# qwerty35/swarm_simulator

Measured on AMD Instinct MI355X. Metric: agent-trajectories/sec (RBP plan: SFC+RSFC+QP), higher is better.
Workload: dtype f64

## Files before the change

### swarm_simulator_amd/csrc/kernels/lh_inverse.inc

```
#define LH_H 3
#include "lh_layout.h"
#define LHP_ZERO 1

__device__ __forceinline__ void lhv_load(const double* x, double (&r)[LH_H], int nP, int lane) {
#pragma unroll
    for (int h = 0; h < LH_H; ++h) r[h] = lane + 64 * h < nP ? x[lane + 64 * h] : 0.0;
}
__device__ __forceinline__ void lhv_store(double* x, const double (&r)[LH_H], int nP, int lane) {
#pragma unroll
    for (int h = 0; h < LH_H; ++h)
        if (lane + 64 * h < nP) x[lane + 64 * h] = r[h];
}
struct LhV {
    double v[LH_H];
};
__device__ __forceinline__ double lhv_pick(const LhV& x, int h) { return h == 0 ? x.v[0] : (h == 1 ? x.v[1] : x.v[2]); }

template <class PT>
__device__ __noinline__ void lh_clear(PT W, int rows_v) {
    const int rows = __builtin_amdgcn_readfirstlane(rows_v);
    const int n = lhp_size(rows);
    for (int i = threadIdx.x & 63; i < n; i += 64) W[i] = 0.0;
    WSYNC();
}

template <int NH, class PT>
__device__ __forceinline__ void w_cols_span(PT W, const LhV& x, double (&out)[LH_H], int g0, int g1, int lane) {
    double A[8][NH], B[8][NH];
    auto load = [&](int g, double (&buf)[8][NH]) {
        const int L = lhp_len(g), base = lhp_grp(g);
#pragma unroll
        for (int h = 0; h < NH; ++h) {
            const int c = lane + 64 * h;
            if (c < L) {
#pragma unroll
                for (int u = 0; u < 8; ++u) buf[u][h] = W[base + u * (L + 1) + c];
            }
        }
    };
    auto use = [&](int g, const double (&buf)[8][NH]) {
        const int L = lhp_len(g);
        const double xs = lhv_pick(x, g >> 3);
        double xb[8];
#pragma unroll
        for (int u = 0; u < 8; ++u) xb[u] = rl_dyn(xs, (8 * g + u) & 63);
#pragma unroll
        for (int h = 0; h < NH; ++h) {
            if (lane + 64 * h < L) {
#pragma unroll
                for (int u = 0; u < 8; ++u) out[h] += buf[u][h] * xb[u];
            }
        }
    };
    if (g0 >= g1) return;
    load(g0, A);
    for (int g = g0; g < g1; g += 2) {
        if (g + 1 < g1) load(g + 1, B);
        use(g, A);
        if (g + 1 < g1) {
            if (g + 2 < g1) load(g + 2, A);
            use(g + 1, B);
        }
    }
}
template <int HM, class PT>
__device__ __noinline__ LhV w_cols_fn(PT W, LhV x, int nP_v) {
    const int nP = __builtin_amdgcn_readfirstlane(nP_v);
    const int lane = threadIdx.x & 63, ng = (nP + 7) >> 3;
    LhV o;
#pragma unroll
    for (int h = 0; h < LH_H; ++h) o.v[h] = 0.0;
    w_cols_span<1, PT>(W, x, o.v, 0, ng < 8 ? ng : 8, lane);
    if (ng > 8) w_cols_span<2, PT>(W, x, o.v, 8, ng < 16 ? ng : 16, lane);
    if (HM > 2 && ng > 16) w_cols_span<(HM > 2 ? 3 : 2), PT>(W, x, o.v, 16, ng, lane);
    return o;
}

template <class PT>
__device__ __noinline__ double w_cols1_fn(PT W, double x0, int nP_v) {
    const int nP = __builtin_amdgcn_readfirstlane(nP_v);
    LhV x, o;
    x.v[0] = x0, x.v[1] = x.v[2] = 0.0;
    o.v[0] = o.v[1] = o.v[2] = 0.0;
    w_cols_span<1, PT>(W, x, o.v, 0, (nP + 7) >> 3, threadIdx.x & 63);
    return o.v[0];
}

template <int H0, int HM, class PT>
__device__ __forceinline__ void w_rows_span(PT W, const LhV& x, double (&out)[LH_H], int g0, int g1, int nP, int lane) {
    constexpr int NH = HM - H0;
    int off[NH], row[NH];
#pragma unroll
    for (int q = 0; q < NH; ++q) {
        const int b = lane + 64 * (H0 + q);
        row[q] = b < nP ? b : -1;
        off[q] = lhp_row(b < nP ? b : 0);
    }
    double A[8][NH], B[8][NH];
    auto load = [&](int g, double (&buf)[8][NH]) {
#pragma unroll
        for (int q = 0; q < NH; ++q) {
            if (row[q] >= 8 * g) {
#pragma unroll
                for (int u = 0; u < 8; ++u) buf[u][q] = W[off[q] + 8 * g + u];
            }
        }
    };
    auto use = [&](int g, const double (&buf)[8][NH]) {
        const double xs = lhv_pick(x, g >> 3);
        double xc[8];
#pragma unroll
        for (int u = 0; u < 8; ++u) xc[u] = rl_dyn(xs, (8 * g + u) & 63);
#pragma unroll
        for (int q = 0; q < NH; ++q) {
            if (row[q] >= 8 * g) {
#pragma unroll
                for (int u = 0; u < 8; ++u) out[H0 + q] += buf[u][q] * xc[u];
            }
        }
    };
    if (g0 >= g1) return;
    load(g0, A);
    for (int g = g0; g < g1; g += 2) {
        if (g + 1 < g1) load(g + 1, B);
        use(g, A);
        if (g + 1 < g1) {
            if (g + 2 < g1) load(g + 2, A);
            use(g + 1, B);
        }
    }
}
template <int HM, class PT>
__device__ __noinline__ LhV w_rows_fn(PT W, LhV x, int nP_v) {
    const int nP = __builtin_amdgcn_readfirstlane(nP_v);
    const int lane = threadIdx.x & 63, ng = (nP + 7) >> 3;
    LhV o;
#pragma unroll
    for (int h = 0; h < LH_H; ++h) o.v[h] = 0.0;
    w_rows_span<0, HM, PT>(W, x, o.v, 0, ng < 8 ? ng : 8, nP, lane);
    if (ng > 8) w_rows_span<1, HM, PT>(W, x, o.v, 8, ng < 16 ? ng : 16, nP, lane);
    if (HM > 2 && ng > 16) w_rows_span<(HM > 2 ? 2 : 1), HM, PT>(W, x, o.v, 16, ng, nP, lane);
    return o;
}
template <class PT>
__device__ __noinline__ double w_rows1_fn(PT W, double x0, int nP_v) {
    const int nP = __builtin_amdgcn_readfirstlane(nP_v);
    const int lane = threadIdx.x & 63, ng = (nP + 7) >> 3;
    const int row = lane < nP ? lane : -1, off = lhp_row(lane < nP ? lane : 0);
    double out = 0.0;
    double A[8], B[8];
    auto load = [&](int g, double (&buf)[8]) {
        if (row >= 8 * g) {
#pragma unroll
            for (int u = 0; u < 8; ++u) buf[u] = W[off + 8 * g + u];
        }
    };
    auto use = [&](int g, const double (&buf)[8]) {
        double xc[8];
#pragma unroll
        for (int u = 0; u < 8; ++u) xc[u] = rl_dyn(x0, 8 * g + u);
        if (row >= 8 * g) {
#pragma unroll
            for (int u = 0; u < 8; ++u) out += buf[u] * xc[u];
        }
    };
    if (ng == 0) return 0.0;
    load(0, A);
    for (int g = 0; g < ng; g += 2) {
        if (g + 1 < ng) load(g + 1, B);
        use(g, A);
        if (g + 1 < ng) {
            if (g + 2 < ng) load(g + 2, A);
            use(g + 1, B);
        }
    }
    return out;
}

template <int H, class PT>
__device__ __noinline__ void w_delete_fn(PT W, double* scr_g, int nP_v, int k_v) {
    const int nP = __builtin_amdgcn_readfirstlane(nP_v), k = __builtin_amdgcn_readfirstlane(k_v);
    const int lane = threadIdx.x & 63;
    kl_lds* scr = (kl_lds*)scr_g;
    double cr[H];
#pragma unroll
    for (int h = 0; h < H; ++h) {
        const int b = lane + 64 * h;
        const bool on = b >= k && b < nP;
        const double v = W[on ? lhp_row(b) + k : LHP_ZERO];
        cr[h] = v;
        if (b < nP) scr[b] = v * v;
    }
    WSYNC();
    double cs[H], sn[H];
    {
        double run[H], prev[H];
#pragma unroll
        for (int h = 0; h < H; ++h) run[h] = 0.0, prev[h] = 0.0;
        for (int r0 = k; r0 < nP; r0 += 8) {
            double q[8];
#pragma unroll
            for (int u = 0; u < 8; ++u) q[u] = scr[r0 + u < nP ? r0 + u : k];
#pragma unroll
            for (int u = 0; u < 8; ++u) {
                const int r = r0 + u < nP ? r0 + u : 1 << 20;
#pragma unroll
                for (int h = 0; h < H; ++h) {
                    run[h] += r <= lane + 64 * h ? q[u] : 0.0;
                    prev[h] += r < lane + 64 * h ? q[u] : 0.0;
                }
            }
        }
#pragma unroll
        for (int h = 0; h < H; ++h) {
            const int i = lane + 64 * h;
            const bool on = i > k && i < nP;
            const double r2 = on ? run[h] : 1.0, p2 = on ? prev[h] : 1.0;
            const double inv = fast_rsqrt(r2);
            cs[h] = on ? p2 * fast_rsqrt(p2) * inv : 1.0;
            sn[h] = on ? cr[h] * inv : 0.0;
        }
    }
    constexpr int DU = 4;
    double acc[H], A[DU][H], B[DU][H];
    int cdst[H];
    auto fetch = [&](int i0, double (&g)[DU][H]) {
#pragma unroll
        for (int u = 0; u < DU; ++u) {
            const int i = i0 + u < nP ? i0 + u : nP - 1;
            const int off = lhp_row(i), len = lhp_len(i >> 3);
#pragma unroll
            for (int h = 0; h < H; ++h) g[u][h] = W[lane + 64 * h < len ? off + lane + 64 * h : LHP_ZERO];
        }
    };
    auto rotate = [&](int i0, const double (&g)[DU][H]) {
#pragma unroll
        for (int u = 0; u < DU; ++u) {
            const int i = i0 + u;
            if (i < nP) {
                const int li = i & 63, hi = i >> 6;
                double ci = rl_dyn(cs[0], li), si = rl_dyn(sn[0], li);
                if (H > 1 && hi == 1) ci = rl_dyn(cs[H > 1 ? 1 : 0], li), si = rl_dyn(sn[H > 1 ? 1 : 0], li);
                if (H > 2 && hi == 2) ci = rl_dyn(cs[H > 2 ? 2 : 0], li), si = rl_dyn(sn[H > 2 ? 2 : 0], li);
                const int tdst = lhp_row(i - 1), ldst = lhp_len((i - 1) >> 3);
#pragma unroll
                for (int h = 0; h < H; ++h) {
                    const double a = acc[h], rv = g[u][h];
                    acc[h] = ci * a + si * rv;
                    const double nv = ci * rv - si * a;
                    if (cdst[h] < ldst) W[tdst + cdst[h]] = nv;
                }
            }
        }
    };
#pragma unroll
    for (int h = 0; h < H; ++h) {
        const int c = lane + 64 * h;
        acc[h] = W[c < lhp_len(k >> 3) ? lhp_row(k) + c : LHP_ZERO];
        cdst[h] = c < k ? c : (c > k ? c - 1 : 1 << 20);
    }
    fetch(k + 1, A);
    for (int i0 = k + 1; i0 < nP; i0 += 2 * DU) {
        if (i0 + DU < nP) fetch(i0 + DU, B);
        rotate(i0, A);
        if (i0 + DU < nP) {
            if (i0 + 2 * DU < nP) fetch(i0 + 2 * DU, A);
            rotate(i0 + DU, B);
        }
    }
    WSYNC();
}

__device__ __forceinline__ void lh_rows(kl_lds* Wl, double* Wg, const double (&x)[LH_H], double (&out)[LH_H], int nP, int lane) {
    if (nP <= 64) {
        out[0] = Wg ? w_rows1_fn<double*>(Wg, x[0], nP) : w_rows1_fn<kl_lds*>(Wl, x[0], nP);
        out[1] = out[2] = 0.0;
        return;
    }
    LhV xi, o;
#pragma unroll
    for (int h = 0; h < LH_H; ++h) xi.v[h] = x[h];
    o = Wg ? w_rows_fn<3, double*>(Wg, xi, nP) : (nP <= 128 ? w_rows_fn<2, kl_lds*>(Wl, xi, nP) : w_rows_fn<3, kl_lds*>(Wl, xi, nP));
#pragma unroll
    for (int h = 0; h < LH_H; ++h) out[h] = o.v[h];
}
__device__ __forceinline__ void lh_cols(kl_lds* Wl, double* Wg, const double (&x)[LH_H], double (&out)[LH_H], int nP, int lane) {
    if (nP <= 64) {
        out[0] = Wg ? w_cols1_fn<double*>(Wg, x[0], nP) : w_cols1_fn<kl_lds*>(Wl, x[0], nP);
        out[1] = out[2] = 0.0;
        return;
    }
    LhV xi, o;
#pragma unroll
    for (int h = 0; h < LH_H; ++h) xi.v[h] = x[h];
    o = Wg ? w_cols_fn<3, double*>(Wg, xi, nP) : (nP <= 128 ? w_cols_fn<2, kl_lds*>(Wl, xi, nP) : w_cols_fn<3, kl_lds*>(Wl, xi, nP));
#pragma unroll
    for (int h = 0; h < LH_H; ++h) out[h] = o.v[h];
}
__device__ __forceinline__ void lh_delete(kl_lds* Wl, double* Wg, double* scr, int nP, int k, int lane) {
    if (Wg)
        w_delete_fn<3, double*>(Wg, scr, nP, k);
    else if (nP <= 64)
        w_delete_fn<1, kl_lds*>(Wl, scr, nP, k);
    else if (nP <= 128)
        w_delete_fn<2, kl_lds*>(Wl, scr, nP, k);
    else
        w_delete_fn<3, kl_lds*>(Wl, scr, nP, k);
}
__device__ __forceinline__ void lh_reset(kl_lds* Wl, double* Wg, int rows) {
    if (Wg)
        lh_clear<double*>(Wg, rows);
    else
        lh_clear<kl_lds*>(Wl, rows);
}
```

### swarm_simulator_amd/csrc/kernels/qp_polish.inc

```

__device__ __forceinline__ int cand_meta(const Cand& c) {
    return c.a | ((c.b + 1) << 8) | ((c.n[0] != 0.0) << 16) | ((c.n[1] != 0.0) << 17) | ((c.n[2] != 0.0) << 18);
}
__device__ __forceinline__ int meta_sign(int meta, int agent, int k) {
    if (!(((meta >> 16) >> k) & 1)) return 0;
    return agent == (meta & 255) ? 1 : (agent == ((meta >> 8) & 255) - 1 ? -1 : 0);
}
__device__ __forceinline__ double cand_dot(const Cand& c, const double* vec, int nk) {
    const double* blk = vec + (size_t)(c.knot - 1) * nk;
    double s = 0;
#pragma unroll
    for (int k = 0; k < 3; ++k) {
        if (c.n[k] == 0.0) continue;
        const double* pa = blk + (c.a * 3 + k) * 3;
        double ta = c.t[0] * pa[0] + c.t[1] * pa[1] + c.t[2] * pa[2];
        if (c.b >= 0) {
            const double* pb = blk + (c.b * 3 + k) * 3;
            ta -= c.t[0] * pb[0] + c.t[1] * pb[1] + c.t[2] * pb[2];
        }
        s += c.n[k] * ta;
    }
    return s;
}

__device__ void k0_mission_tables(int nj, const QpWs& w, const PolishWs& pw, double* lds) {
    double* f3 = lds;
    dd* fd = (dd*)(lds + 18 * nj);
    for (int it = threadIdx.x; it < 18 * nj; it += QP_THREADS) {
        const int jj = it / 18, e = it % 18, j = jj + 1;
        const double v = e < 9 ? w.Dk[9 * j + e] : (jj + 1 < nj ? w.Ek[9 * j + (e - 9)] : 0.0);
        f3[it] = v, fd[it] = dd(v);
    }
    __syncthreads();
    if (threadIdx.x == 0) {
        int ok = 1;
        double Bp[9] = {0, 0, 0, 0, 0, 0, 0, 0, 0};
        for (int jj = 0; jj < nj; ++jj)
            if (!k0_factor_step(f3 + 18 * jj, Bp, jj == 0)) ok = 0;
        *(int*)(pw.k0f + 18 * (size_t)nj) = !ok;
    }
    if (threadIdx.x == 64) {
        int ok = 1;
        dd Bd[9];
        for (int jj = 0; jj < nj; ++jj)
            if (!k0_factor_step(fd + 18 * jj, Bd, jj == 0)) ok = 0;
        *((int*)(pw.k0f + 18 * (size_t)nj) + 1) = !ok;
    }
    __syncthreads();
    for (int it = threadIdx.x; it < 18 * nj; it += QP_THREADS) pw.k0f[it] = f3[it];
    for (int col = threadIdx.x; col < 3 * nj; col += QP_THREADS) k0_inverse_column((const dd*)fd, nj, col / 3, col % 3, pw.G, pw.Sg);
    __threadfence_block();
    __syncthreads();
    for (int jj = threadIdx.x; jj < nj; jj += QP_THREADS) k0g_symmetrise(pw.G + k0g_block(jj, jj));
}

__device__ __forceinline__ void k0_solve3(const double* f3g, int nj, int nk, double* col, int sub) {
    typedef __attribute__((address_space(1))) double gdb;
    const kl_lds* f3 = (const kl_lds*)f3g;
    gdb* y = QG(col) + sub * 3;
    constexpr int B = K0_BLK;
    double cur[B][3], nxt[B][3];
    double p[3] = {0, 0, 0};
#pragma unroll
    for (int u = 0; u < B; ++u) {
        const int jx = u < nj ? u : nj - 1;
#pragma unroll
        for (int e = 0; e < 3; ++e) cur[u][e] = y[(size_t)jx * nk + e];
    }
    for (int j0 = 0; j0 < nj; j0 += B) {
#pragma unroll
        for (int u = 0; u < B; ++u) {
            const int jx = j0 + B + u < nj ? j0 + B + u : nj - 1;
#pragma unroll
            for (int e = 0; e < 3; ++e) nxt[u][e] = y[(size_t)jx * nk + e];
        }
#pragma unroll
        for (int u = 0; u < B; ++u) {
            const int jj = j0 + u;
            if (jj < nj) {
                k0_forward_step(f3 + 18 * jj, jj > 0, cur[u], p);
                y[(size_t)jj * nk] = p[0] = cur[u][0], y[(size_t)jj * nk + 1] = p[1] = cur[u][1], y[(size_t)jj * nk + 2] = p[2] = cur[u][2];
            }
        }
#pragma unroll
        for (int u = 0; u < B; ++u)
#pragma unroll
            for (int e = 0; e < 3; ++e) cur[u][e] = nxt[u][e];
    }
#pragma unroll
    for (int u = 0; u < B; ++u) {
        const int jx = nj - 1 - u >= 0 ? nj - 1 - u : 0;
#pragma unroll
        for (int e = 0; e < 3; ++e) cur[u][e] = y[(size_t)jx * nk + e];
    }
    for (int jt = nj - 1; jt >= 0; jt -= B) {
#pragma unroll
        for (int u = 0; u < B; ++u) {
            const int jx = jt - B - u >= 0 ? jt - B - u : 0;
#pragma unroll
            for (int e = 0; e < 3; ++e) nxt[u][e] = y[(size_t)jx * nk + e];
        }
#pragma unroll
        for (int u = 0; u < B; ++u) {
            const int jj = jt - u;
            if (jj >= 0) {
                k0_backward_step(f3 + 18 * jj, jj + 1 < nj, cur[u], p);
                y[(size_t)jj * nk] = p[0] = cur[u][0], y[(size_t)jj * nk + 1] = p[1] = cur[u][1], y[(size_t)jj * nk + 2] = p[2] = cur[u][2];
            }
        }
#pragma unroll
        for (int u = 0; u < B; ++u)
#pragma unroll
            for (int e = 0; e < 3; ++e) cur[u][e] = nxt[u][e];
    }
}

__device__ __noinline__ void v0_solve3_fn(int nj_v, int nk_v, int nb_v, double* v0_v, const double* f3_v) {
    const int nj = __builtin_amdgcn_readfirstlane(nj_v), nk = __builtin_amdgcn_readfirstlane(nk_v), nb = __builtin_amdgcn_readfirstlane(nb_v);
    double* v0 = uni(v0_v);
    const double* f3 = uni(f3_v);
    for (int it = threadIdx.x; it < nb * 3; it += QP_THREADS) k0_solve3(f3, nj, nk, v0, it);
}

__device__ __noinline__ void table_product_fn(int nj_v, int nk_v, int nb_v, const double* G_v, const double* u_v, double* out_v) {
    typedef __attribute__((address_space(1))) const double gcd;
    const int nj = __builtin_amdgcn_readfirstlane(nj_v), nk = __builtin_amdgcn_readfirstlane(nk_v), nsub = 3 * __builtin_amdgcn_readfirstlane(nb_v);
    gcd* G = QGC(uni(G_v));
    gcd* uv = QGC(uni(u_v));
    double* out = uni(out_v);
    constexpr int PB = 4;
    for (int it = threadIdx.x; it < nj * nsub; it += QP_THREADS) {
        const int jj = it / nsub, sub = it % nsub;
        double acc[3] = {0, 0, 0};
        for (int k0 = 0; k0 < nj; k0 += PB) {
            double g[PB][9], x[PB][3];
#pragma unroll
            for (int u = 0; u < PB; ++u) {
                const int kb = k0 + u < nj ? k0 + u : nj - 1;
                gcd* blk = G + (jj >= kb ? k0g_block(jj, kb) : k0g_block(kb, jj));
#pragma unroll
                for (int e = 0; e < 9; ++e) g[u][e] = blk[e];
#pragma unroll
                for (int e = 0; e < 3; ++e) x[u][e] = uv[(size_t)kb * nk + sub * 3 + e];
            }
#pragma unroll
            for (int u = 0; u < PB; ++u) {
                if (k0 + u >= nj) continue;
                if (jj >= k0 + u) {
                    acc[0] += g[u][0] * x[u][0] + g[u][1] * x[u][1] + g[u][2] * x[u][2];
                    acc[1] += g[u][3] * x[u][0] + g[u][4] * x[u][1] + g[u][5] * x[u][2];
                    acc[2] += g[u][6] * x[u][0] + g[u][7] * x[u][1] + g[u][8] * x[u][2];
                } else {
                    acc[0] += g[u][0] * x[u][0] + g[u][3] * x[u][1] + g[u][6] * x[u][2];
                    acc[1] += g[u][1] * x[u][0] + g[u][4] * x[u][1] + g[u][7] * x[u][2];
                    acc[2] += g[u][2] * x[u][0] + g[u][5] * x[u][1] + g[u][8] * x[u][2];
                }
            }
        }
        const size_t i = (size_t)jj * nk + sub * 3;
#pragma unroll
        for (int e = 0; e < 3; ++e) out[i + e] = -acc[e];
    }
}

__device__ __forceinline__ double s_from_table(const Cand* cand, const double* G, int ci, int cj, int ma, int mb) {
    const int aa = ma & 255, ab = ((ma >> 8) & 255) - 1, ba = mb & 255, bb = ((mb >> 8) & 255) - 1;
    const int sg = (aa == ba) - (bb >= 0 && aa == bb) - (ab >= 0 && ab == ba) + (ab >= 0 && ab == bb);
    bool share = aa == ba || (bb >= 0 && aa == bb) || (ab >= 0 && (ab == ba || ab == bb));
    if (share && ab < 0 && bb < 0) share = ((ma & mb) >> 16) != 0;
    if (!share || sg == 0) return 0.0;
    const Cand& ca = cand[ci];
    const Cand& cb = cand[cj];
    const bool a_first = ca.knot >= cb.knot;
    const double* blk = G + k0g_block((a_first ? ca.knot : cb.knot) - 1, (a_first ? cb.knot : ca.knot) - 1);
    return (double)sg * (ca.n[0] * cb.n[0] + ca.n[1] * cb.n[1] + ca.n[2] * cb.n[2]) * k0g_bilinear(blk, a_first, ca.t, cb.t);
}

__device__ __forceinline__ double rl_dyn(double v, int lane) {
    const int lo = __builtin_amdgcn_readlane(__double2loint(v), lane);
    const int hi = __builtin_amdgcn_readlane(__double2hiint(v), lane);
    return __hiloint2double(hi, lo);
}

#include "lh_inverse.inc"

__device__ int lh_wave(int n, const double* Sg, int ldS, const double* dv, double* zc, double* tv, double* yv, double* wv, int* P, int* inP,
                       int* banned, double* Lc, int* shared_int, int pmax, double* str, bool big, double* stats = nullptr, int resume_nP = -1,
                       int n_prev = 0) {
    const int lane = threadIdx.x & 63;
    kl_lds* Wl = big ? nullptr : (kl_lds*)Lc;
    double* Wg = big ? Lc : nullptr;
    int* rem = (int*)tv;
    int nP = 0;
    double dmax = 0;
    const bool resume = resume_nP >= 0;
    for (int a = lane; a < n; a += 64) {
        if (!resume || a >= n_prev)
            zc[a] = 0;
        else
            zc[a] = fmax(zc[a], 0.0);
        inP[a] = 0, banned[a] = 0;
        dmax = fmax(dmax, fabs(dv[a]));
    }
    dmax = wave_red(dmax, 1);
    const double wtol = 1e-12 * fmax(1.0, dmax);
    if (resume) {
        nP = resume_nP;
        WSYNC();
        for (int b = lane; b < nP; b += 64) inP[P[b]] = 1;
    } else {
        lh_reset(Wl, Wg, pmax);
    }
    WSYNC();
    bool warming = str != nullptr && !resume;
    bool w_valid = resume ? shared_int[1] != 0 : true;
    bool first_resumed = resume && nP > 0;
    if (stats && lane == 0) stats[7] += 1.0;
    for (int itn = 0; itn < 6 * n + 20; ++itn) {
        long long lt0 = stats ? wall_clock64() : 0;
        double best = wtol;
        int bidx = -1;
        bool do_append = true;
        if (first_resumed) {
            first_resumed = false, do_append = false;
        } else if (warming) {
            best = 100.0;
            for (int a = lane; a < n; a += 64)
                if (str[a] > best) best = str[a], bidx = a;
            wave_argmax(best, bidx);
            if (bidx >= 0 && lane == 0) str[bidx] = 0.0;
            WSYNC();
            if (bidx < 0 || nP >= pmax - 8) {
                warming = false, do_append = false;
                if (nP == 0) continue;
            }
        } else {
            double acc[4] = {0, 0, 0, 0};
            for (int q0 = 0; q0 < nP; q0 += 64) {
                const int pl = q0 + lane < nP ? P[q0 + lane] : -1;
                const double zl = pl >= 0 ? zc[pl] : 0.0;
                const int nb = nP - q0 < 64 ? nP - q0 : 64;
                for (int b0 = 0; b0 < nb; b0 += 4) {
                    double sv[4][4], zb[4];
#pragma unroll
                    for (int u = 0; u < 4; ++u) {
                        const int bb = b0 + u < nb ? b0 + u : nb - 1;
                        const int pb = __builtin_amdgcn_readlane(pl, bb);
                        zb[u] = b0 + u < nb ? rl_dyn(zl, bb) : 0.0;
                        const double* row = Sg + (size_t)pb * ldS;
#pragma unroll
                        for (int v = 0; v < 4; ++v) sv[u][v] = lane + 64 * v < n ? row[lane + 64 * v] : 0.0;
                    }
#pragma unroll
                    for (int u = 0; u < 4; ++u)
#pragma unroll
                        for (int v = 0; v < 4; ++v) acc[v] += sv[u][v] * zb[u];
                }
            }
#pragma unroll
            for (int v = 0; v < 4; ++v) {
                const int a = lane + 64 * v;
                if (a < n) {
                    const double s = dv[a] - acc[v];
                    if (!inP[a] && !banned[a] && s > best) best = s, bidx = a;
                }
            }
            wave_argmax(best, bidx);
            if (stats && lane == 0) { const long long t_ = wall_clock64(); stats[0] += (double)(t_ - lt0); lt0 = t_; stats[4] += 1.0; }
            if (bidx < 0) break;
        }
        const int j = bidx;
        if (do_append) {
            if (nP >= pmax) return -1;
            double sr[LH_H], lr[LH_H], wr[LH_H], tr[LH_H];
#pragma unroll
            for (int h = 0; h < LH_H; ++h) sr[h] = lane + 64 * h < nP ? Sg[(size_t)P[lane + 64 * h] * ldS + j] : 0.0;
            lh_rows(Wl, Wg, sr, lr, nP, lane);
            lhv_load(wv, wr, nP, lane);
            double ll = 0, lw = 0;
#pragma unroll
            for (int h = 0; h < LH_H; ++h) ll += lr[h] * lr[h], lw += w_valid ? lr[h] * wr[h] : 0.0;
            ll = wave_red(ll, 0);
            const double sjj = Sg[(size_t)j * ldS + j];
            const double djj = sjj - ll;
            if (!(djj > 1e-13 * fmax(1e-30, sjj))) {
                if (lane == 0) banned[j] = 1;
                WSYNC();
                continue;
            }
            lw = wave_red(lw, 0);
            lh_cols(Wl, Wg, lr, tr, nP, lane);
            const double ir = fast_rsqrt(djj);
            {
                const int rowo = lhp_row(nP), len = lhp_len(nP >> 3);
#pragma unroll
                for (int h = 0; h < LH_H; ++h) {
                    const int cq = lane + 64 * h;
                    if (cq < len) Lc[rowo + cq] = cq < nP ? -ir * tr[h] : (cq == nP ? ir : 0.0);
                }
            }
            if (lane == 0) {
                P[nP] = j;
                inP[j] = 1;
                wv[nP] = (dv[j] - lw) * ir;
            }
            nP++;
            WSYNC();
            if (stats && lane == 0) { const long long t_ = wall_clock64(); stats[1] += (double)(t_ - lt0); lt0 = t_; stats[5] += 1.0; }
        }
        if (warming) continue;
        for (int inner = 0; inner < 2 * pmax; ++inner) {
            {
                double wr[LH_H], yr[LH_H];
                if (!w_valid) {
                    double dr[LH_H];
#pragma unroll
                    for (int h = 0; h < LH_H; ++h) dr[h] = lane + 64 * h < nP ? dv[P[lane + 64 * h]] : 0.0;
                    lh_rows(Wl, Wg, dr, wr, nP, lane);
                    lhv_store(wv, wr, nP, lane);
                    w_valid = true;
                } else
                    lhv_load(wv, wr, nP, lane);
                lh_cols(Wl, Wg, wr, yr, nP, lane);
                lhv_store(yv, yr, nP, lane);
                WSYNC();
                if (stats && lane == 0) stats[6] += 1.0;
            }
            double ymin = 1e300;
            for (int b = lane; b < nP; b += 64) ymin = fmin(ymin, yv[b]);
            ymin = wave_red(ymin, 2);
            if (ymin > 0) {
                for (int b = lane; b < nP; b += 64) zc[P[b]] = yv[b];
                WSYNC();
                if (stats && lane == 0) { const long long t_ = wall_clock64(); stats[2] += (double)(t_ - lt0); lt0 = t_; }
                break;
            }
            double alpha = 1e300;
            for (int b = lane; b < nP; b += 64)
                if (yv[b] <= 0) alpha = fmin(alpha, zc[P[b]] / (zc[P[b]] - yv[b]));
            alpha = wave_red(alpha, 2);
            if (stats && lane == 0) { const long long t_ = wall_clock64(); stats[2] += (double)(t_ - lt0); lt0 = t_; }
            if (!(alpha >= 0)) alpha = 0;
            for (int b = lane; b < nP; b += 64) zc[P[b]] += alpha * (yv[b] - zc[P[b]]);
            WSYNC();
            if (lane == 0) {
                int nrem = 0, worst = 0;
                for (int b = 1; b < nP; ++b)
                    if (yv[b] < yv[worst]) worst = b;
                for (int b = 0; b < nP; ++b) {
                    const int ia = P[b];
                    if (yv[b] <= 0 && zc[ia] <= 1e-14 * fmax(1.0, fabs(yv[b]))) rem[nrem++] = b;
                }
                if (nrem == 0) rem[nrem++] = worst;
                *shared_int = nrem;
            }
            WSYNC();
            const int nrem = *shared_int;
            for (int q = nrem - 1; q >= 0; --q) {
                const int pos = rem[q];
                lh_delete(Wl, Wg, yv, nP, pos, lane);
                if (lane == 0) {
                    const int ia = P[pos];
                    zc[ia] = 0, inP[ia] = 0;
                    for (int b = pos; b < nP - 1; ++b) P[b] = P[b + 1];
                }
                nP--;
                WSYNC();
            }
            for (int a = lane; a < n; a += 64) banned[a] = 0;
            w_valid = false;
            WSYNC();
            if (stats && lane == 0) { const long long t_ = wall_clock64(); stats[3] += (double)(t_ - lt0); lt0 = t_; }
            if (nP == 0) break;
        }
    }
    if (lane == 0) shared_int[1] = w_valid ? 1 : 0;
    return nP;
}

__device__ __forceinline__ int polish_qp(RowCtx& c, PassIO& io, const PolishWs& pw, double* lds, double* red, int* flag, int mode) {
    const bool geometric = mode == 1, big = mode == 2;
    const QpDims& d = c.d;
    const QpWs& w = c.w;
    const int tid = threadIdx.x, NK = d.nk;
    double* ctrl = const_cast<double*>(c.ctrl);
    const int pmax = big ? PL_PBIG : polish_pmax(NK);
    double* Lc = big ? pw.Lbig : lds;
    double* zc = big ? lds : lds + lhp_size(pmax);
    double* dv = zc + PL_NC;
    double* tv = dv + PL_NC;
    double* yv = tv + pmax;
    double* wv = yv + pmax;
    int* P = (int*)(wv + pmax);
    int* inP = P + pmax;
    int* banned = inP + PL_NC;
    int* sint = banned + PL_NC;
    double* str = (double*)(sint + 4);
    double* f3 = str + PL_NC;

#ifdef QP_LHSTATS
#define QP_PPROF_ON 0
#else
#define QP_PPROF_ON 1
#endif
#ifdef QP_PROFILE
    double* pscal = c.scal + 20;
    long long pt0 = wall_clock64();
#define PPROF(i)                                       \
    do {                                               \
        __syncthreads();                               \
        const long long t_ = wall_clock64();           \
        if (tid == 0 && QP_PPROF_ON) pscal[i] += (double)(t_ - pt0);  \
        pt0 = t_;                                      \
    } while (0)
#else
#define PPROF(i)
#endif
    if (tid == 0) pw.ncand[0] = 0;
    __threadfence_block();
    __syncthreads();
    if (geometric)
        row_pass<PASS_CAND_GEO>(c, io);
    else
        row_pass<PASS_CAND>(c, io);
    __threadfence_block();
    __syncthreads();
    if (pw.ncand[0] > PL_NC) return 1;

    {
        const int* k0bad = (const int*)(pw.k0f + 18 * (size_t)d.nj);
        if (k0bad[0] | k0bad[1]) return 2;
    }
    for (int it = tid; it < 18 * d.nj; it += QP_THREADS) f3[it] = pw.k0f[it];

    for (int it0 = tid; it0 < d.nb * 3 * d.oq; it0 += 4 * QP_THREADS) {
        double xq[4][6], sc4[4];
#pragma unroll
        for (int q = 0; q < 4; ++q) {
            const int it = it0 + q * QP_THREADS < d.nb * 3 * d.oq ? it0 + q * QP_THREADS : it0;
            const int a = it / (3 * d.oq), k = (it / d.oq) % 3, j6 = it % d.oq, m = j6 / 6;
            const double* xs = ctrl + ((size_t)(d.first + a) * 3 + k) * d.oq + 6 * m;
#pragma unroll
            for (int jj = 0; jj < 6; ++jj) xq[q][jj] = xs[jj];
            sc4[q] = w.segsc[m];
        }
#pragma unroll
        for (int q = 0; q < 4; ++q) {
            const int it = it0 + q * QP_THREADS;
            if (it < d.nb * 3 * d.oq) {
                const int i = (it % d.oq) % 6;
                double g = 0;
#pragma unroll
                for (int jj = 0; jj < 6; ++jj) g += Qbase[6 * i + jj] * xq[q][jj];
                w.cvec[it] = 2 * sc4[q] * g;
            }
        }
    }
    __threadfence_block();
    __syncthreads();
    double* gred = pw.v0 + (size_t)d.nj * NK;
    double* usum = gred + (size_t)d.nj * NK;
    apply_FT(d, w, w.cvec, gred, 1.0);
    __threadfence_block();
    __syncthreads();
    for (int i = tid; i < d.nj * NK; i += QP_THREADS) pw.v0[i] = gred[i];
    __threadfence_block();
    __syncthreads();
    v0_solve3_fn(d.nj, d.nk, d.nb, pw.v0, f3);
    __threadfence_block();
    __syncthreads();

    PPROF(0);
    bool accepted = false;
    int n_done = 0, nP = 0;
    for (int outer = 0; outer < 8 && !accepted; ++outer) {
        const int n = pw.ncand[0];
        if (n > PL_NC) return 1;
        const int n_prev = n_done;
#ifndef QP_PROFILE
        if (outer > 0 && tid == 0) c.scal[SC_PROF0 + 4] += 1;
#endif
        const int first_new = n_done;
        {
            const int n_new = n - first_new;
            for (int i = tid; i < n_new; i += QP_THREADS) inP[i] = pw.cand[first_new + i].row;
            __syncthreads();
            Cand mine;
            int rank = 0;
            if (tid < n_new) {
                mine = pw.cand[first_new + tid];
                for (int j = 0; j < n_new; ++j) rank += inP[j] < mine.row;
            }
            __syncthreads();
            if (tid < n_new) pw.cand[first_new + rank] = mine;
            __threadfence_block();
            __syncthreads();
        }
        for (int ci = tid; ci < n; ci += QP_THREADS) inP[ci] = cand_meta(pw.cand[ci]);
        n_done = n;
        __syncthreads();
        for (int it = tid; it < n * n; it += QP_THREADS) {
            const int ci = it / n, cj = it % n;
            if (cj > ci || ci < first_new) continue;
            const double sv = s_from_table(pw.cand, pw.G, ci, cj, inP[ci], inP[cj]);
            pw.Sg[(size_t)ci * PL_NC + cj] = sv;
            pw.Sg[(size_t)cj * PL_NC + ci] = sv;
        }
        for (int ci = tid; ci < n; ci += QP_THREADS) dv[ci] = -cand_dot(pw.cand[ci], pw.v0, NK) - pw.cand[ci].slack;
        for (int ci = tid; ci < n; ci += QP_THREADS)
            str[ci] = outer == 0 ? pw.cand[ci].strength : (ci < n_prev && zc[ci] > 0 ? 1e3 + zc[ci] : 0.0);
        __threadfence_block();
        __syncthreads();
        const double* Suse = pw.Sg;
        int ldS = PL_NC;
        {
            double* Sl = f3 + 18 * d.nj;
            if ((int)(Sl - lds) + n * n <= c.lds_avail) {
                for (int it = tid; it < n * n; it += QP_THREADS) Sl[it] = pw.Sg[(size_t)(it / n) * PL_NC + it % n];
                Suse = Sl, ldS = n;
                __syncthreads();
            }
        }
        PPROF(1);
        if (tid < 64) {
            __builtin_amdgcn_s_setprio(QP_CHAIN_PRIO);
            const int res_nP = (outer > 0 && nP > 0) ? nP : -1;
#ifdef QP_LHSTATS
            const int r = lh_wave(n, Suse, ldS, dv, zc, tv, yv, wv, P, inP, banned, Lc, sint + 2, pmax, str, big, c.scal + 20, res_nP, n_prev);
#else
            const int r = lh_wave(n, Suse, ldS, dv, zc, tv, yv, wv, P, inP, banned, Lc, sint + 2, pmax, str, big, nullptr, res_nP, n_prev);
#endif
            __builtin_amdgcn_s_setprio(0);
            if (tid == 0) sint[1] = r;
        }
        __syncthreads();
        nP = sint[1];
        PPROF(2);
        if (nP < 0) return 3;
        int* pmeta = inP;
        int* off = banned;
        const int nsub = 3 * d.nb;
        for (int b = tid; b < nP; b += QP_THREADS) pmeta[b] = cand_meta(pw.cand[P[b]]);
        __syncthreads();
        for (int sub = tid; sub < nsub; sub += QP_THREADS) {
            int cnt = 0;
            for (int b = 0; b < nP; ++b) cnt += meta_sign(pmeta[b], sub / 3, sub % 3) != 0;
            ((int*)str)[sub] = cnt;
        }
        __syncthreads();
        for (int sub = tid; sub <= nsub; sub += QP_THREADS) {
            int o = 0;
            for (int q = 0; q < sub; ++q) o += ((int*)str)[q];
            off[sub] = o;
        }
        __syncthreads();
        for (int it = tid; it < nP * 6; it += QP_THREADS) {
            const int b = it / 6, side = (it % 6) / 3, k = it % 3;
            const int meta = pmeta[b], ag = side == 0 ? (meta & 255) : ((meta >> 8) & 255) - 1;
            if (ag < 0 || !(((meta >> 16) >> k) & 1)) continue;
            int rank = 0;
            for (int q = 0; q < b; ++q) rank += meta_sign(pmeta[q], ag, k) != 0;
            const Cand& cd = pw.cand[P[b]];
            const double sn = side == 0 ? cd.n[k] : -cd.n[k];
            double* en = pw.ptab + 4 * (size_t)(off[ag * 3 + k] + rank);
            en[0] = (double)((cd.knot - 1) * 1024 + b), en[1] = sn * cd.t[0], en[2] = sn * cd.t[1], en[3] = sn * cd.t[2];
        }
        __threadfence_block();
        __syncthreads();
        for (int round = 0; round < 4; ++round) {
            for (int b = tid; b < nP; b += QP_THREADS) tv[b] = zc[P[b]];
            __syncthreads();
            for (int it = tid; it < d.nj * nsub; it += QP_THREADS) {
                const int kb = it / nsub, sub = it % nsub;
                const size_t i = (size_t)kb * NK + sub * 3;
                double u0 = gred[i], u1 = gred[i + 1], u2 = gred[i + 2];
                for (int o = off[sub]; o < off[sub + 1]; ++o) {
                    const double* en = pw.ptab + 4 * (size_t)o;
                    const int key = (int)en[0];
                    if ((key >> 10) == kb) {
                        const double zb = tv[key & 1023];
                        u0 += zb * en[1], u1 += zb * en[2], u2 += zb * en[3];
                    }
                }
                usum[i] = u0, usum[i + 1] = u1, usum[i + 2] = u2;
            }
            __threadfence_block();
            __syncthreads();
            table_product_fn(d.nj, NK, d.nb, pw.G, usum, w.rhs);
            __threadfence_block();
            __syncthreads();
            apply_F(d, w, w.rhs, w.dx);
            __threadfence_block();
            __syncthreads();
            io.vmax = 0;
            row_pass<PASS_VERIFY>(c, io);
            const double vmax = block_reduce(io.vmax, 1, red);
            __threadfence_block();
            __syncthreads();
            if (pw.ncand[0] > n) break;
            double emax = 0, zmin = 0, zmax = 0;
            for (int b = tid; b < nP; b += QP_THREADS) {
                const double e = w.ds[pw.cand[P[b]].row];
                yv[b] = -e;
                emax = fmax(emax, fabs(e));
                zmin = fmin(zmin, zc[P[b]]), zmax = fmax(zmax, zc[P[b]]);
            }
            emax = block_reduce(emax, 1, red);
            zmin = block_reduce(zmin, 2, red);
            zmax = block_reduce(zmax, 1, red);
#ifdef QP_POLSTATS
            if (tid == 0) {
                double* ps = c.scal + 20;
                ps[0] = vmax, ps[1] = zmin, ps[2] = zmax, ps[3] = emax + 1000.0 * round + 1e6 * outer + 1e8 * nP + 1e12 * n;
            }
#endif
            if (vmax <= 5e-9 && zmin >= -1e-9 * fmax(1.0, zmax) && (emax < 1e-12 || round == 3)) {
                accepted = true;
                if (tid == 0) red[12] = fmax(fmax(vmax, 0.0), fmax(0.0, -zmin) / fmax(1.0, zmax));
                break;
            }
            if (round == 3) break;
            if (tid < 64 && nP > 0) {
                const int lane = tid;
                double er[LH_H], ur[LH_H], yr[LH_H];
                kl_lds* Wl = big ? nullptr : (kl_lds*)Lc;
                double* Wg = big ? Lc : nullptr;
                lhv_load(yv, er, nP, lane);
                lh_rows(Wl, Wg, er, ur, nP, lane);
                lh_cols(Wl, Wg, ur, yr, nP, lane);
#pragma unroll
                for (int h = 0; h < LH_H; ++h)
                    if (lane + 64 * h < nP) zc[P[lane + 64 * h]] += yr[h];
            }
            __syncthreads();
        }
        PPROF(3);
        if (!accepted && pw.ncand[0] <= n) break;
    }
    if (!accepted) return 4;
    {
        double* xb = ctrl + (size_t)d.first * 3 * d.oq;
        const int nx = d.nb * 3 * d.oq;
        for (int i0 = tid; i0 < nx; i0 += 4 * QP_THREADS) {
            double xv[4], dv4[4];
#pragma unroll
            for (int q = 0; q < 4; ++q) {
                const int i = i0 + q * QP_THREADS;
                xv[q] = i < nx ? xb[i] : 0.0, dv4[q] = i < nx ? w.dx[i] : 0.0;
            }
#pragma unroll
            for (int q = 0; q < 4; ++q)
                if (i0 + q * QP_THREADS < nx) xb[i0 + q * QP_THREADS] = xv[q] + dv4[q];
        }
    }
    __threadfence_block();
    __syncthreads();
    for (int b = tid; b < nP; b += QP_THREADS) {
        const Cand& cd = pw.cand[P[b]];
        if (cd.snap_idx >= 0 && zc[P[b]] > 0) ctrl[cd.snap_idx] = cd.snap_val;
    }
    __threadfence_block();
    __syncthreads();
    return 0;
}

__device__ __noinline__ int polish_entry(RowCtx c_in, PolishWs pw_in, double* lds, double* red, int* flag, int mode) {
    PassIO io = {};
    RowCtx c = uni_words(c_in);
    PolishWs pw = uni_words(pw_in);
    c.pw = &pw;
    return polish_qp(c, io, pw, uni(lds), uni(red), uni(flag), uni(mode));
}
```

Measured before the change: 197,100.

## Add blocked 8-column warm-start append to the LH inverse in QP polish

Warm-start constraints in the active-set QP are now ranked once up front instead of re-scanned with a wave argmax on every iteration. When the active set size is a multiple of 8, they are appended eight at a time using a blocked Schur-complement update: an 8x8 Cholesky factor plus matrix-matrix products over the LDS inverse. This replaces eight rank-1 append iterations with one blocked step, cutting per-iteration synchronisation and memory passes. It adds register pressure and new code paths, and if a pivot fails mid-block it bans that constraint and falls back to the single-append path.

```diff
diff --git a/swarm_simulator_amd/csrc/kernels/lh_block.h b/swarm_simulator_amd/csrc/kernels/lh_block.h
--- /dev/null
+++ b/swarm_simulator_amd/csrc/kernels/lh_block.h
@@ -0,0 +1,78 @@
+#pragma once
+#include "lh_layout.h"
+#ifndef LHB_FN
+#define LHB_FN __host__ __device__ inline
+#endif
+#if defined(__clang__)
+#define LHB_UNROLL _Pragma("unroll")
+#else
+#define LHB_UNROLL
+#endif
+#define LHB 8
+
+LHB_FN bool lhb_fits(int nP, int left, int pmax) { return (nP & 7) == 0 && left >= LHB && nP + 2 * LHB <= pmax; }
+LHB_FN int lhb_scr(int g) { return lhp_grp(g + 1); }
+LHB_FN int lhb_at(int r, int u) { return LHB * r + u; }
+#define LHB_NSUM 44
+LHB_FN int lhb_tri(int a, int b) { return a * (a + 1) / 2 + b; }
+LHB_FN void lhb_sum_of(int e, int& a, int& b) {
+    if (e >= 36) {
+        a = e - 36, b = LHB;
+        return;
+    }
+    a = 0;
+    while (lhb_tri(a + 1, 0) <= e) ++a;
+    b = e - lhb_tri(a, 0);
+}
+template <class PX, class PY>
+LHB_FN double lhb_dot(PX x, int sx, PY y, int sy, int rows) {
+    double s0 = 0, s1 = 0, s2 = 0, s3 = 0;
+    for (int r = 0; r < rows; r += 4) {
+        s0 += x[r * sx] * y[r * sy];
+        s1 += x[(r + 1) * sx] * y[(r + 1) * sy];
+        s2 += x[(r + 2) * sx] * y[(r + 2) * sy];
+        s3 += x[(r + 3) * sx] * y[(r + 3) * sy];
+    }
+    return (s0 + s1) + (s2 + s3);
+}
+LHB_FN bool lhb_before(double sa, int a, double sb, int b) { return sa > sb || (sa == sb && a < b); }
+
+struct LhBlock {
+    double c[LHB][LHB];
+    int good;
+};
+template <class RS>
+LHB_FN void lhb_factor(LhBlock& B, const double (&sd)[LHB], RS rs) {
+    int good = LHB;
+    LHB_UNROLL
+    for (int k = 0; k < LHB; ++k) {
+        double p = B.c[k][k];
+        LHB_UNROLL
+        for (int m = 0; m < k; ++m) p -= B.c[k][m] * B.c[k][m];
+        const bool ok = good == LHB && p > 1e-13 * fmax(1e-30, sd[k]);
+        if (!ok && good == LHB) good = k;
+        const double ir = ok ? rs(p) : 1.0;
+        B.c[k][k] = ir;
+        LHB_UNROLL
+        for (int i = k + 1; i < LHB; ++i) {
+            double s = B.c[i][k];
+            LHB_UNROLL
+            for (int m = 0; m < k; ++m) s -= B.c[i][m] * B.c[k][m];
+            B.c[i][k] = ok ? s * ir : 0.0;
+        }
+    }
+    B.good = good;
+}
+LHB_FN void lhb_solve(const double (&gp)[36], double (&y)[LHB]) {
+    LHB_UNROLL
+    for (int a = 0; a < LHB; ++a) {
+        double s = y[a];
+        LHB_UNROLL
+        for (int b = 0; b < a; ++b) s -= gp[a * (a + 1) / 2 + b] * y[b];
+        y[a] = s * gp[a * (a + 1) / 2 + a];
+    }
+}
+#define LHB_SCR_V 36
+#define LHB_SCR_GI LHB_NSUM
+#define LHB_SCR_SD (LHB_SCR_GI + 36)
+#define LHB_SCR (LHB_SCR_SD + LHB)
diff --git a/swarm_simulator_amd/csrc/kernels/lh_inverse.inc b/swarm_simulator_amd/csrc/kernels/lh_inverse.inc
--- a/swarm_simulator_amd/csrc/kernels/lh_inverse.inc
+++ b/swarm_simulator_amd/csrc/kernels/lh_inverse.inc
@@ -313,3 +313,239 @@
     else
         lh_clear<kl_lds*>(Wl, rows);
 }
+
+#ifndef LH_BLOCK_WARM
+#define LH_BLOCK_WARM 1
+#endif
+#define LHB_FN __host__ __device__ __forceinline__
+#include "lh_block.h"
+#define LHB_SCHED() __builtin_amdgcn_sched_barrier(0)
+
+template <class T>
+__device__ __forceinline__ T* lh_uni(T* p) {
+    const unsigned long long v = (unsigned long long)p;
+    const unsigned lo = __builtin_amdgcn_readfirstlane((unsigned)v), hi = __builtin_amdgcn_readfirstlane((unsigned)(v >> 32));
+    return (T*)(((unsigned long long)hi << 32) | lo);
+}
+
+__device__ __forceinline__ void w_rows8(kl_lds* W, kl_lds* X, double (&out)[LHB], int q, int ng, int lane) {
+    const int b = lane + 64 * q;
+    const int row = b < 8 * ng ? b : -1, off = lhp_row(b < 8 * ng ? b : 0);
+    const int g1 = q == 0 && ng > 8 ? 8 : ng;
+    double A[8], B[8];
+    auto load = [&](int g, double (&buf)[8]) {
+#pragma unroll
+        for (int u = 0; u < 8; ++u) buf[u] = W[row >= 8 * g ? off + 8 * g + u : LHP_ZERO];
+    };
+    auto use = [&](int g, const double (&buf)[8]) {
+#pragma unroll
+        for (int u = 0; u < 8; ++u) {
+            double x[LHB];
+#pragma unroll
+            for (int e = 0; e < LHB; ++e) x[e] = X[lhb_at(8 * g + u, e)];
+#pragma unroll
+            for (int e = 0; e < LHB; ++e) out[e] += buf[u] * x[e];
+            if (u & 1) LHB_SCHED();
+        }
+    };
+    if (g1 <= 0) return;
+    load(0, A);
+    for (int g = 0; g < g1; g += 2) {
+        if (g + 1 < g1) load(g + 1, B);
+        use(g, A);
+        if (g + 1 < g1) {
+            if (g + 2 < g1) load(g + 2, A);
+            use(g + 1, B);
+        }
+    }
+}
+__device__ __forceinline__ void w_cols8(kl_lds* W, kl_lds* X, double (&out)[LHB], int h, int ng, int lane) {
+    const int c = lane + 64 * h;
+    const int g0 = h == 0 ? 0 : 8;
+    double A[8], B[8];
+    auto load = [&](int g, double (&buf)[8]) {
+        const int L = lhp_len(g), base = lhp_grp(g);
+#pragma unroll
+        for (int u = 0; u < 8; ++u) buf[u] = W[c < L ? base + u * (L + 1) + c : LHP_ZERO];
+    };
+    auto use = [&](int g, const double (&buf)[8]) {
+#pragma unroll
+        for (int u = 0; u < 8; ++u) {
+            double x[LHB];
+#pragma unroll
+            for (int e = 0; e < LHB; ++e) x[e] = X[lhb_at(8 * g + u, e)];
+#pragma unroll
+            for (int e = 0; e < LHB; ++e) out[e] += buf[u] * x[e];
+            if (u & 1) LHB_SCHED();
+        }
+    };
+    if (g0 >= ng) return;
+    load(g0, A);
+    for (int g = g0; g < ng; g += 2) {
+        if (g + 1 < ng) load(g + 1, B);
+        use(g, A);
+        if (g + 1 < ng) {
+            if (g + 2 < ng) load(g + 2, A);
+            use(g + 1, B);
+        }
+    }
+}
+
+__device__ __noinline__ int lh_block_step_fn(double* scr_v) {
+    double* scr = lh_uni(scr_v);
+    LhBlock B;
+    double sd[LHB];
+#pragma unroll
+    for (int a = 0; a < LHB; ++a) {
+#pragma unroll
+        for (int b = 0; b < LHB; ++b) B.c[a][b] = b <= a ? scr[lhb_tri(a, b)] : 0.0;
+        sd[a] = scr[LHB_SCR_SD + a];
+    }
+    lhb_factor(B, sd, [](double x) { return fast_rsqrt(x); });
+    if ((threadIdx.x & 63) == 0) {
+#pragma unroll
+        for (int a = 0; a < LHB; ++a)
+#pragma unroll
+            for (int b = 0; b <= a; ++b) scr[LHB_SCR_GI + lhb_tri(a, b)] = B.c[a][b];
+    }
+    return __builtin_amdgcn_readfirstlane(B.good);
+}
+
+template <int NH>
+__device__ __noinline__ int w_block_fn(kl_lds* W, const double* Sg_v, int ldS_v, int* P_v, const int* Jl_v, const double* dv_v, double* wv_v,
+                                       int* inP_v, double* scr_v, int nP_v) {
+    const int nP = __builtin_amdgcn_readfirstlane(nP_v), ldS = __builtin_amdgcn_readfirstlane(ldS_v);
+    const double* Sg = lh_uni(Sg_v);
+    const double* dv = lh_uni(dv_v);
+    double* wv = lh_uni(wv_v);
+    double* scr = lh_uni(scr_v);
+    int* P = lh_uni(P_v);
+    int* inP = lh_uni(inP_v);
+    const int* Jl = lh_uni(Jl_v);
+    const int lane = threadIdx.x & 63, ng = nP >> 3;
+    kl_lds* X = W + lhb_scr(ng);
+    int J[LHB];
+#pragma unroll
+    for (int u = 0; u < LHB; ++u) J[u] = __builtin_amdgcn_readfirstlane(Jl[u]);
+#pragma unroll
+    for (int q = 0; q < NH; ++q) {
+        const int c = lane + 64 * q;
+        if (c < nP) {
+            const double* srow = Sg + (size_t)P[c] * ldS;
+#pragma unroll
+            for (int u = 0; u < LHB; ++u) X[lhb_at(c, u)] = srow[J[u]];
+        }
+    }
+    WSYNC();
+    {
+        double Lr[LHB][NH];
+#pragma unroll
+        for (int u = 0; u < LHB; ++u)
+#pragma unroll
+            for (int q = 0; q < NH; ++q) Lr[u][q] = 0.0;
+#pragma unroll
+        for (int q = 0; q < NH; ++q) {
+            double o[LHB];
+#pragma unroll
+            for (int u = 0; u < LHB; ++u) o[u] = 0.0;
+            w_rows8(W, X, o, q, ng, lane);
+#pragma unroll
+            for (int u = 0; u < LHB; ++u) Lr[u][q] = o[u];
+        }
+        WSYNC();
+#pragma unroll
+        for (int q = 0; q < NH; ++q) {
+            const int b = lane + 64 * q;
+            if (b < nP) {
+#pragma unroll
+                for (int u = 0; u < LHB; ++u) X[lhb_at(b, u)] = Lr[u][q];
+            }
+        }
+    }
+    WSYNC();
+    if (lane < LHB_NSUM) {
+        int a, b;
+        lhb_sum_of(lane, a, b);
+        const int ja = Jl[a];
+        double s;
+        if (b < LHB) {
+            const double sab = Sg[(size_t)ja * ldS + Jl[b]];
+            if (a == b) scr[LHB_SCR_SD + a] = sab;
+            s = sab - lhb_dot(X + a, LHB, X + b, LHB, nP);
+        } else
+            s = dv[ja] - lhb_dot(X + a, LHB, (kl_lds*)wv, 1, nP);
+        scr[lane] = s;
+    }
+    WSYNC();
+    const int good = lh_block_step_fn(scr);
+    double T[LHB][NH];
+#pragma unroll
+    for (int u = 0; u < LHB; ++u)
+#pragma unroll
+        for (int h = 0; h < NH; ++h) T[u][h] = 0.0;
+#pragma unroll
+    for (int h = 0; h < NH; ++h) {
+        double o[LHB];
+#pragma unroll
+        for (int u = 0; u < LHB; ++u) o[u] = 0.0;
+        w_cols8(W, X, o, h, ng, lane);
+#pragma unroll
+        for (int u = 0; u < LHB; ++u) T[u][h] = o[u];
+    }
+    WSYNC();
+    {
+        double gp[36];
+#pragma unroll
+        for (int e = 0; e < 36; ++e) gp[e] = scr[LHB_SCR_GI + e];
+#pragma unroll
+        for (int h = 0; h <= NH; ++h) {
+            double y[LHB];
+#pragma unroll
+            for (int b = 0; b < LHB; ++b) y[b] = h < NH ? -T[b][h < NH ? h : 0] : (lane == LHB ? scr[LHB_SCR_V + b] : (lane == b ? 1.0 : 0.0));
+            lhb_solve(gp, y);
+            const int c = h < NH ? lane + 64 * h : nP + lane;
+            const bool on = h < NH ? c < nP : lane < LHB;
+#pragma unroll
+            for (int a = 0; a < LHB; ++a) {
+                if (a < good) {
+                    if (on) W[lhp_row(nP + a) + c] = y[a];
+                    if (h == NH && lane == LHB) wv[nP + a] = y[a];
+                }
+            }
+        }
+        if (lane == 0) {
+#pragma unroll
+            for (int a = 0; a < LHB; ++a)
+                if (a < good) P[nP + a] = J[a], inP[J[a]] = 1;
+        }
+    }
+    WSYNC();
+    return good;
+}
+__device__ __noinline__ int lh_rank_warm(const double* str_v, int n_v, int* list_v, int cap_v) {
+    const int n = __builtin_amdgcn_readfirstlane(n_v), cap = __builtin_amdgcn_readfirstlane(cap_v);
+    const double* str = lh_uni(str_v);
+    int* list = lh_uni(list_v);
+    const int lane = threadIdx.x & 63;
+    double ms[4];
+    int rk[4] = {0, 0, 0, 0}, nw = 0;
+#pragma unroll
+    for (int v = 0; v < 4; ++v) ms[v] = lane + 64 * v < n ? str[lane + 64 * v] : 0.0;
+    for (int b = 0; b < n; ++b) {
+        const double sb = str[b];
+        if (sb > 100.0) {
+            nw++;
+#pragma unroll
+            for (int v = 0; v < 4; ++v) rk[v] += lhb_before(sb, b, ms[v], lane + 64 * v) ? 1 : 0;
+        }
+    }
+#pragma unroll
+    for (int v = 0; v < 4; ++v)
+        if (ms[v] > 100.0 && rk[v] < cap) list[rk[v]] = lane + 64 * v;
+    WSYNC();
+    return __builtin_amdgcn_readfirstlane(nw < cap ? nw : cap);
+}
+__device__ __forceinline__ int lh_block(kl_lds* Wl, const double* Sg, int ldS, int* P, const int* Jl, const double* dv, double* wv, int* inP,
+                                        double* scr, int nP) {
+    return nP <= 64 ? w_block_fn<1>(Wl, Sg, ldS, P, Jl, dv, wv, inP, scr, nP) : w_block_fn<2>(Wl, Sg, ldS, P, Jl, dv, wv, inP, scr, nP);
+}
diff --git a/swarm_simulator_amd/csrc/kernels/qp_polish.inc b/swarm_simulator_amd/csrc/kernels/qp_polish.inc
--- a/swarm_simulator_amd/csrc/kernels/qp_polish.inc
+++ b/swarm_simulator_amd/csrc/kernels/qp_polish.inc
@@ -216,6 +216,11 @@
     bool w_valid = resume ? shared_int[1] != 0 : true;
     bool first_resumed = resume && nP > 0;
     if (stats && lane == 0) stats[7] += 1.0;
+#if LH_BLOCK_WARM
+    const bool listed = warming && !big;
+    int nw = 0, wq = 0;
+    if (listed) nw = lh_rank_warm(str, n, rem, 2 * pmax);
+#endif
     for (int itn = 0; itn < 6 * n + 20; ++itn) {
         long long lt0 = stats ? wall_clock64() : 0;
         double best = wtol;
@@ -223,6 +228,26 @@
         bool do_append = true;
         if (first_resumed) {
             first_resumed = false, do_append = false;
+#if LH_BLOCK_WARM
+        } else if (warming && listed) {
+            if (wq >= nw || nP >= pmax - 8) {
+                warming = false, do_append = false;
+                if (nP == 0) continue;
+            } else if (lhb_fits(nP, nw - wq, pmax)) {
+                const int good = lh_block(Wl, Sg, ldS, P, rem + wq, dv, wv, inP, yv, nP);
+                nP += good;
+                if (good < LHB) {
+                    if (lane == 0) banned[rem[wq + good]] = 1;
+                    WSYNC();
+                }
+                wq += good < LHB ? good + 1 : LHB;
+                if (stats && lane == 0) stats[8] += (double)(wall_clock64() - lt0), stats[9] += 1.0, stats[10] += (double)good;
+                continue;
+            } else {
+                bidx = __builtin_amdgcn_readfirstlane(rem[wq]);
+                wq++;
+            }
+#endif
         } else if (warming) {
             best = 100.0;
             for (int a = lane; a < n; a += 64)
```

Result: no change. 198,300, median of 3 (+0.6%).
